# ForJadeForest/DistillCLIP

Measured on AMD Instinct MI355X. Metric: image-text pairs/sec (distill step), higher is better.
Workload: dtype bf16; 1 GPU; l_clip.yaml dual distill: ViT-B/32 CLIP teacher -> weight-shared ViT(6x768,24h,R2) + text(4x768,12h,R2) students, 224px/77tok, losses out_l1+out_cos+0.1*cos_diff, fwd+loss+bwd+AdamW; global_batch=512, batch_per_gpu=512, parallelism=dp1, gradient_exchange=none, negatives=local (reference training_step semantics), optimizer_in_step=True, teacher_residual=fp16, saved_gelu_derivative=u8 fixed point, clock_probe=True

## Files before the change

### distillclip_amd/_lib.py

```python
import ctypes
import os
import re

_HERE = os.path.dirname(os.path.abspath(__file__))
_LIB_PATH = os.path.join(_HERE, 'libdistillclip_hip.so')
_HEADER = os.path.join(os.path.dirname(_HERE), 'include', 'dclip.h')

_CT = {
    "int32_t": ctypes.c_int32,
    'int': ctypes.c_int, 'int64_t': ctypes.c_int64, 'float': ctypes.c_float, 'size_t': ctypes.c_size_t,
    'double': ctypes.c_double, 'dclip_bucket_cb': ctypes.c_void_p,
}


def _parse_header(path=_HEADER):
    src = open(path).read()
    src = re.sub(r'/\*.*?\*/', '', src, flags=re.S)
    src = re.sub(r'//[^\n]*', '', src)
    src = re.sub(r'^\s*#[^\n]*$', '', src, flags=re.M)
    src = src.replace('extern "C" {', '')
    src = re.sub(r'typedef\s+struct[^;{]*\{.*?\}[^;]*;', '', src, flags=re.S)
    src = re.sub(r'typedef[^;]*;', '', src)
    protos = {}
    for m in re.finditer(r'((?:const\s+)?(?:int|void|char|float|size_t|int64_t|int32_t|dclip_encoder)[\s\*]*?)\b(dclip_\w+)\s*\(([^)]*)\)\s*;', src):
        ret, name, args = m.group(1).strip(), m.group(2), m.group(3).strip()
        protos[name] = (_ctype(ret), [] if args in ('', 'void') else [_ctype(a) for a in args.split(',')])
    return protos


def _ctype(decl):
    decl = decl.strip()
    if '*' in decl:
        return ctypes.c_char_p if re.match(r'const\s+char\s*\*', decl) and decl.count('*') == 1 and \
            not re.search(r'\*\s*\w+$', decl) else ctypes.c_void_p
    toks = [t for t in re.split(r'\s+', decl) if t not in ('const', 'unsigned', 'struct')]
    return None if toks[0] == 'void' else _CT[toks[0]]


class DclipError(RuntimeError):
    pass


class _Lib:
    def __init__(self):
        if not os.path.exists(_LIB_PATH):
            raise ImportError(
                f'{_LIB_PATH} is missing: build it with `python -c "import __graft_entry__ as g; g.build()"` '
                f'(or `make -C distillclip_amd/csrc`).  distillclip_amd has no CPU fallback.')
        import torch
        self._dll = ctypes.CDLL(_LIB_PATH)
        self.protos = _parse_header()
        for name, (res, args) in self.protos.items():
            fn = getattr(self._dll, name)
            fn.restype = res
            fn.argtypes = args
        if self._dll.dclip_arch() != b'gfx950':
            raise ImportError('libdistillclip_hip.so was not built for gfx950')

    def __getattr__(self, name):
        fn = getattr(self._dll, name)
        if self.protos.get(name, (None,))[0] is not ctypes.c_int or name in ('dclip_version', 'dclip_encoder_num_grad_buckets') or name.endswith('_supported'):
            return fn

        def call(*args):
            rc = fn(*args)
            if rc != 0:
                msg = self._dll.dclip_last_error_string().decode()
                if rc == -1:
                    raise ValueError(msg)
                raise DclipError(f'{name} failed ({rc}): {msg}')
        call.__name__ = name
        setattr(self, name, call)
        return call


_lib = None


def lib():
    global _lib
    if _lib is None:
        _lib = _Lib()
    return _lib
```

### distillclip_amd/csrc/layernorm.hip

```cpp
#include <stdlib.h>
#include "common.h"

namespace {

constexpr int LN_MAXV = 4;

template <int NV, int OUT, bool X_F16>
__global__ __launch_bounds__(256) void ln_fwd_kernel(const void* __restrict__ x, int64_t ldx, const int* __restrict__ ridx,
                                                     const float* __restrict__ gamma, const float* __restrict__ beta,
                                                     void* __restrict__ y, int64_t ldy, float* __restrict__ mean,
                                                     float* __restrict__ rstd, int M, int D, float eps) {
    const int lane = threadIdx.x & 63;
    const int row = blockIdx.x * 4 + (threadIdx.x >> 6);
    if (row >= M) return;
    const int64_t src = ridx ? ridx[row] : row;
    float4 v[NV];
    float s = 0.f;
#pragma unroll
    for (int i = 0; i < NV; ++i) {
        const int c = (i * 64 + lane) * 4;
        v[i] = float4{0.f, 0.f, 0.f, 0.f};
        if (c < D) {
            if (X_F16) {
                const f16x4 h = *(const f16x4*)((const _Float16*)x + src * ldx + c);
                v[i] = float4{(float)h[0], (float)h[1], (float)h[2], (float)h[3]};
            } else {
                v[i] = *(const float4*)((const float*)x + src * ldx + c);
            }
        }
        s += (v[i].x + v[i].y) + (v[i].z + v[i].w);
    }
    const float mu = wave_sum(s) / D;
    float q = 0.f;
#pragma unroll
    for (int i = 0; i < NV; ++i) {
        const int c = (i * 64 + lane) * 4;
        if (c < D) {
            const float a = v[i].x - mu, b = v[i].y - mu, cc = v[i].z - mu, d = v[i].w - mu;
            q += (a * a + b * b) + (cc * cc + d * d);
        }
    }
    const float rs = rsqrtf(wave_sum(q) / D + eps);
    if (lane == 0) {
        if (mean) mean[row] = mu;
        if (rstd) rstd[row] = rs;
    }
#pragma unroll
    for (int i = 0; i < NV; ++i) {
        const int c = (i * 64 + lane) * 4;
        if (c < D) {
            const float4 g = *(const float4*)(gamma + c), b = *(const float4*)(beta + c);
            const float o0 = (v[i].x - mu) * rs * g.x + b.x, o1 = (v[i].y - mu) * rs * g.y + b.y;
            const float o2 = (v[i].z - mu) * rs * g.z + b.z, o3 = (v[i].w - mu) * rs * g.w + b.w;
            if (OUT == 1) {
                *(float4*)((float*)y + (int64_t)row * ldy + c) = float4{o0, o1, o2, o3};
            } else if (OUT == 2) {
                *(f16x4*)((_Float16*)y + (int64_t)row * ldy + c) = f16x4{(_Float16)o0, (_Float16)o1, (_Float16)o2, (_Float16)o3};
            } else {
                bf16x4 o = {f2bf(o0), f2bf(o1), f2bf(o2), f2bf(o3)};
                *(bf16x4*)((bf16_t*)y + (int64_t)row * ldy + c) = o;
            }
        }
    }
}

template <int NV, bool DY_F32>
__global__ __launch_bounds__(512) void ln_bwd_kernel(const void* __restrict__ dy, int64_t lddy, const float* __restrict__ x,
                                                     int64_t ldx, const int* __restrict__ ridx,
                                                     const float* __restrict__ gamma, const float* __restrict__ mean,
                                                     const float* __restrict__ rstd, float* __restrict__ dx_acc,
                                                     int64_t lddx, bf16_t* __restrict__ dx_bf16, int64_t lddb,
                                                     float* __restrict__ dgamma, float* __restrict__ dbeta, float* __restrict__ colsum, int M, int D) {
    constexpr int NW = 8, DP = NV * 256;
    extern __shared__ float red_[];
    float (*red)[NW][DP] = (float (*)[NW][DP])red_;
    const int lane = threadIdx.x & 63, wave = threadIdx.x >> 6;
    float4 dg[NV], db[NV], gm[NV], cs[NV];
#pragma unroll
    for (int i = 0; i < NV; ++i) {
        dg[i] = db[i] = cs[i] = float4{0.f, 0.f, 0.f, 0.f};
        const int c = (i * 64 + lane) * 4;
        gm[i] = c < D ? *(const float4*)(gamma + c) : float4{0.f, 0.f, 0.f, 0.f};
    }
    struct Raw {
        float4 x[NV], a[NV], d[NV];
        float mu, rs;
        int64_t src;
        int row;
    };
    auto issue = [&](int row, Raw& r) {
        r.row = row;
        r.src = ridx ? ridx[row] : row;
        r.mu = mean[row];
        r.rs = rstd[row];
#pragma unroll
        for (int i = 0; i < NV; ++i) {
            const int c = (i * 64 + lane) * 4;
            r.x[i] = r.a[i] = r.d[i] = float4{0.f, 0.f, 0.f, 0.f};
            if (c < D) {
                r.x[i] = *(const float4*)(x + r.src * ldx + c);
                r.a[i] = *(const float4*)(dx_acc + r.src * lddx + c);
                if (DY_F32) r.d[i] = *(const float4*)((const float*)dy + (int64_t)row * lddy + c);
                else {
                    const bf16x4 t = *(const bf16x4*)((const bf16_t*)dy + (int64_t)row * lddy + c);
                    union { bf16x4 h; float2 f; } u; u.h = t;
                    r.d[i].x = u.f.x; r.d[i].y = u.f.y;
                }
            }
        }
    };
    auto process = [&](const Raw& r) {
        float4 xh[NV], g[NV];
        float s1 = 0.f, s2 = 0.f;
#pragma unroll
        for (int i = 0; i < NV; ++i) {
            const int c = (i * 64 + lane) * 4;
            xh[i] = g[i] = float4{0.f, 0.f, 0.f, 0.f};
            if (c < D) {
                float4 d;
                if (DY_F32) d = r.d[i];
                else {
                    union { bf16x4 h; float2 f; } u; u.f = float2{r.d[i].x, r.d[i].y};
                    d = float4{bf2f(u.h[0]), bf2f(u.h[1]), bf2f(u.h[2]), bf2f(u.h[3])};
                }
                const float4 xv = r.x[i];
                xh[i] = float4{(xv.x - r.mu) * r.rs, (xv.y - r.mu) * r.rs, (xv.z - r.mu) * r.rs, (xv.w - r.mu) * r.rs};
                g[i] = float4{d.x * gm[i].x, d.y * gm[i].y, d.z * gm[i].z, d.w * gm[i].w};
                s1 += (g[i].x + g[i].y) + (g[i].z + g[i].w);
                s2 += (g[i].x * xh[i].x + g[i].y * xh[i].y) + (g[i].z * xh[i].z + g[i].w * xh[i].w);
                dg[i].x += d.x * xh[i].x; dg[i].y += d.y * xh[i].y; dg[i].z += d.z * xh[i].z; dg[i].w += d.w * xh[i].w;
                db[i].x += d.x; db[i].y += d.y; db[i].z += d.z; db[i].w += d.w;
            }
        }
        const float c1 = wave_sum(s1) / D, c2 = wave_sum(s2) / D;
#pragma unroll
        for (int i = 0; i < NV; ++i) {
            const int c = (i * 64 + lane) * 4;
            if (c < D) {
                float* o = dx_acc + r.src * lddx + c;
                float4 a = r.a[i];
                a.x += r.rs * (g[i].x - c1 - xh[i].x * c2);
                a.y += r.rs * (g[i].y - c1 - xh[i].y * c2);
                a.z += r.rs * (g[i].z - c1 - xh[i].z * c2);
                a.w += r.rs * (g[i].w - c1 - xh[i].w * c2);
                *(float4*)o = a;
                cs[i].x += a.x; cs[i].y += a.y; cs[i].z += a.z; cs[i].w += a.w;
                if (dx_bf16) {
                    bf16x4 bq = {f2bf(a.x), f2bf(a.y), f2bf(a.z), f2bf(a.w)};
                    *(bf16x4*)(dx_bf16 + r.src * lddb + c) = bq;
                }
            }
        }
    };
    const int stride = gridDim.x * NW;
    Raw ra, rb;
    int row = blockIdx.x * NW + wave;
    if (row < M) issue(row, ra);
    while (row < M) {
        int nrow = row + stride;
        if (nrow < M) issue(nrow, rb);
        process(ra);
        row = nrow;
        if (row >= M) break;
        nrow = row + stride;
        if (nrow < M) issue(nrow, ra);
        process(rb);
        row = nrow;
    }
#pragma unroll
    for (int i = 0; i < NV; ++i) {
        const int c = (i * 64 + lane) * 4;
        *(float4*)&red[0][wave][c] = dg[i];
        *(float4*)&red[1][wave][c] = db[i];
        *(float4*)&red[2][wave][c] = cs[i];
    }
    __syncthreads();
    for (int c = threadIdx.x; c < D; c += 64 * NW) {
        float a = 0.f, b = 0.f, k = 0.f;
#pragma unroll
        for (int w = 0; w < NW; ++w) { a += red[0][w][c]; b += red[1][w][c]; k += red[2][w][c]; }
        if (dgamma) unsafeAtomicAdd(dgamma + c, a);
        if (dbeta) unsafeAtomicAdd(dbeta + c, b);
        if (colsum) unsafeAtomicAdd(colsum + c, k);
    }
}

}

#define LN_DISPATCH(NVV, ...)                     \
    switch (NVV) {                                \
        case 1: { constexpr int NV = 1; __VA_ARGS__; break; } \
        case 2: { constexpr int NV = 2; __VA_ARGS__; break; } \
        case 3: { constexpr int NV = 3; __VA_ARGS__; break; } \
        default: { constexpr int NV = 4; __VA_ARGS__; break; } \
    }

static int ln_fwd_launch(const void* x, int x_f16, int64_t ldx, const int32_t* row_index, const float* gamma, const float* beta, void* y,
                         int64_t ldy, int out, float* mean, float* rstd, int64_t M, int64_t D, float eps, void* stream, const char* who) {
    DCLIP_REQUIRE(x && gamma && beta && y, "%s: null operand", who);
    DCLIP_REQUIRE(M > 0 && D > 0 && D % 4 == 0 && D <= 1024, "%s: need 0 < D <= 1024, D %% 4 == 0 (D=%ld)", who, (long)D);
    DCLIP_REQUIRE(ldx % 4 == 0 && ldy % 4 == 0 && ((uintptr_t)x % (x_f16 ? 8 : 16)) == 0, "%s: row strides must be multiples of 4, rows 8- (fp16) / 16-byte aligned", who);
    DCLIP_REQUIRE(out >= 0 && out <= 2 && (out != 2 || x_f16), "%s: output dtype 0 bf16 / 1 f32 (/ 2 f16 with f16 input)", who);
    const int nv = (int)((D + 255) / 256);
    const dim3 grid((unsigned)((M + 3) / 4));
    hipStream_t st = (hipStream_t)stream;
    TraceScope tr(DCLIP_TRACE_LAYERNORM, 8.0 * (double)M * D, (double)M * D * ((x_f16 ? 2.0 : 4.0) + (out == 1 ? 4.0 : 2.0)), stream);
#define LN_GO(OUTV, XH) hipLaunchKernelGGL((ln_fwd_kernel<NV, OUTV, XH>), grid, dim3(256), 0, st, x, ldx, row_index, gamma, beta, y, ldy, mean, rstd, (int)M, (int)D, eps)
    LN_DISPATCH(nv,
        if (x_f16) { if (out == 2) LN_GO(2, true); else if (out == 1) LN_GO(1, true); else LN_GO(0, true); }
        else { if (out == 1) LN_GO(1, false); else LN_GO(0, false); });
#undef LN_GO
    return dclip_check_launch(who);
}

extern "C" int dclip_layernorm_fwd(const float* x, int64_t ldx, const int32_t* row_index, const float* gamma,
                                   const float* beta, void* y, int64_t ldy, int out_f32, float* mean, float* rstd,
                                   int64_t M, int64_t D, float eps, void* stream) {
    return ln_fwd_launch(x, 0, ldx, row_index, gamma, beta, y, ldy, out_f32 ? 1 : 0, mean, rstd, M, D, eps, stream, "dclip_layernorm_fwd");
}

extern "C" int dclip_layernorm_fwd_f16(const void* x, int64_t ldx, const int32_t* row_index, const float* gamma,
                                       const float* beta, void* y, int64_t ldy, int out_dtype, float* mean, float* rstd,
                                       int64_t M, int64_t D, float eps, void* stream) {
    return ln_fwd_launch(x, 1, ldx, row_index, gamma, beta, y, ldy, out_dtype, mean, rstd, M, D, eps, stream, "dclip_layernorm_fwd_f16");
}

extern "C" int dclip_layernorm_bwd(const void* dy, int64_t lddy, int dy_f32, const float* x, int64_t ldx,
                                   const int32_t* row_index, const float* gamma, const float* mean, const float* rstd,
                                   float* dx_acc, int64_t lddx, void* dx_bf16, int64_t lddb, float* dgamma, float* dbeta,
                                   float* colsum_acc, int64_t M, int64_t D, void* stream) {
    DCLIP_REQUIRE(dy && x && gamma && mean && rstd && dx_acc, "dclip_layernorm_bwd: null operand");
    DCLIP_REQUIRE(M > 0 && D > 0 && D % 4 == 0 && D <= 1024, "dclip_layernorm_bwd: need 0 < D <= 1024, D %% 4 == 0 (D=%ld)", (long)D);
    const int nv = (int)((D + 255) / 256);
    int blocks = (int)((M + 7) / 8);
    if (blocks > 256) blocks = 256;
    TraceScope tr(DCLIP_TRACE_LN_BWD, 12.0 * (double)M * D, (double)M * D * ((dy_f32 ? 4.0 : 2.0) + 12.0 + (dx_bf16 ? 2.0 : 0.0)), stream, (int)M, (int)D, 0, 0);
    hipStream_t st = (hipStream_t)stream;
    LN_DISPATCH(nv,
        if (dy_f32) hipLaunchKernelGGL((ln_bwd_kernel<NV, true>), dim3(blocks), dim3(512), (size_t)3 * 8 * NV * 256 * 4, st, dy, lddy, x, ldx, row_index, gamma, mean, rstd, dx_acc, lddx, (bf16_t*)dx_bf16, lddb, dgamma, dbeta, colsum_acc, (int)M, (int)D);
        else hipLaunchKernelGGL((ln_bwd_kernel<NV, false>), dim3(blocks), dim3(512), (size_t)3 * 8 * NV * 256 * 4, st, dy, lddy, x, ldx, row_index, gamma, mean, rstd, dx_acc, lddx, (bf16_t*)dx_bf16, lddb, dgamma, dbeta, colsum_acc, (int)M, (int)D));
    return dclip_check_launch("dclip_layernorm_bwd");
}
```

### include/dclip.h

```cpp
#ifndef DCLIP_H
#define DCLIP_H
#include <stddef.h>
#include <stdint.h>
#ifdef __cplusplus
extern "C" {
#endif

#define DCLIP_OK 0
#define DCLIP_EINVAL (-1)
#define DCLIP_ELAUNCH (-2)

int dclip_version(void);
int dclip_runtime_check(void);
const char* dclip_arch(void);
const char* dclip_last_error_string(void);

#define DCLIP_ACT_NONE 0
#define DCLIP_ACT_QUICKGELU 1
#define DCLIP_ACT_GELU 2
#define DCLIP_ACT_DGELU 3
#define DCLIP_ACT_MULAUX 4
#define DCLIP_ACT_GELU_SAVE 5
#define DCLIP_ACT_QUICKGELU_SAVE 6
#define DCLIP_OUT_BF16 0
#define DCLIP_OUT_F32 1
#define DCLIP_OUT_F16 2

int dclip_gemm_nt(const void* A, int64_t lda, const void* B, int64_t ldb, void* C, int64_t ldc,
                  int64_t M, int64_t N, int64_t K, float alpha, const float* bias, int act,
                  const void* aux_in, void* aux_out, const void* residual, int64_t ldr, int out_dtype,
                  int64_t row_group, const float* rowadd, float* colsum_acc, void* stream);

size_t dclip_gemm_tn_workspace_bytes(void);
int64_t dclip_gemm_tn_atomic_fallbacks(void);
int dclip_gemm_tn_acc(const void* A, int64_t lda, const void* B, int64_t ldb, float* dW, int64_t ldo,
                      int64_t M, int64_t P, int64_t Q, int splits, void* workspace, size_t ws_bytes, void* stream);

int dclip_colsum_acc(const void* X, int64_t ld, float* db, int64_t M, int64_t N, void* stream);

int dclip_layernorm_fwd(const float* x, int64_t ldx, const int32_t* row_index, const float* gamma, const float* beta,
                        void* y, int64_t ldy, int out_f32, float* mean, float* rstd, int64_t M, int64_t D, float eps,
                        void* stream);
int dclip_layernorm_fwd_f16(const void* x, int64_t ldx, const int32_t* row_index, const float* gamma, const float* beta,
                            void* y, int64_t ldy, int out_dtype, float* mean, float* rstd, int64_t M, int64_t D, float eps,
                            void* stream);
int dclip_layernorm_bwd(const void* dy, int64_t lddy, int dy_f32, const float* x, int64_t ldx, const int32_t* row_index,
                        const float* gamma, const float* mean, const float* rstd, float* dx_acc, int64_t lddx,
                        void* dx_bf16, int64_t lddb, float* dgamma, float* dbeta, float* colsum_acc, int64_t M, int64_t D,
                        void* stream);

int dclip_attn_nt(const void* A, int64_t lda, const void* Bm, int64_t ldb, void* C, int out_f32, int64_t B, int64_t H,
                  int64_t N, int64_t Np, int64_t hd, float alpha, void* stream);
int dclip_attn_nn(const void* A, const void* Bm, int64_t ldb, void* C, int64_t ldc, int64_t B, int64_t H, int64_t N,
                  int64_t Np, int64_t hd, float alpha, int a_blocked, void* stream);
int dclip_attn_tn(const void* A, const void* Bm, int64_t ldb, void* C, int64_t ldc, int64_t B, int64_t H, int64_t N,
                  int64_t Np, int64_t hd, float alpha, int a_blocked, void* stream);
int dclip_attn_fused_fwd(const void* qkv, int64_t ldq, void* ctx, int64_t ldc, int64_t B, int64_t H, int64_t N, int64_t hd,
                         float scale, int causal, void* stream);
int dclip_attn_stream_fwd(const void* qkv, int64_t ldq, void* ctx, int64_t ldc, int64_t B, int64_t H, int64_t N, int64_t hd,
                          float scale, void* stream);
int dclip_attn_softmax_fwd(const float* S, const float* Wl, const float* Ww, void* P, void* R, int64_t B, int64_t H,
                           int64_t N, int64_t Np, int causal, void* stream);
int dclip_attn_softmax_bwd(const void* dR, const void* P, const void* S, int scores_bf16, const float* Wl, const float* Ww,
                           void* dS, float* dWl, float* dWw, int64_t B, int64_t H, int64_t N, int64_t Np, void* stream);
int dclip_attn_mix_supported(int64_t H, int64_t N, int64_t hd);
size_t dclip_attn_mix_bwd_workspace_bytes(int64_t B, int64_t H, int64_t N);
void dclip_attn_mix_debug_stamps(void* fwd, void* bwd_a, void* bwd_b);
int dclip_attn_mix_fwd(const void* qkv, int64_t ld, const float* Wl, const float* Ww, void* R, float* stats, int64_t B, int64_t H,
                       int64_t N, int64_t Np, int64_t hd, float scale, void* stream);
int dclip_attn_mix_bwd(const void* qkv, int64_t ld, const void* dO, int64_t ldo, const float* Wl, const float* Ww,
                       const float* stats, void* dS, float* dWl, float* dWw, void* workspace, size_t ws_bytes, int64_t B, int64_t H,
                       int64_t N, int64_t Np, int64_t hd, float scale, void* stream);
int dclip_attn_maps_fwd(const void* qkv, int64_t ld, const float* Wl, float* score_map, float* prob_map, int64_t B, int64_t H, int64_t N,
                        int64_t hd, float scale, int causal, void* stream);
size_t dclip_attn_maps_bwd_workspace_bytes(int64_t B, int64_t H, int64_t N);
int dclip_attn_maps_bwd(const void* qkv, int64_t ld, const float* Wl, const float* d_score_map, const float* d_prob_map, void* dS,
                        int ds_blocked, float* dWl, void* workspace, size_t ws_bytes, int64_t B, int64_t H, int64_t N, int64_t Np,
                        int64_t hd, float scale, int causal, void* stream);

int dclip_cast_bf16(const float* src, void* dst, int64_t n, void* stream);
int dclip_cast_f16_f32(const void* src, float* dst, int64_t n, void* stream);
int dclip_axpy_f32(float* dst, const float* src, void* dst_bf16, int64_t n, float* colsum_acc, int64_t D, void* stream);
int dclip_cast_transpose_bf16_multi(const float* const* W, void* const* Wb, void* const* Wt, const int64_t* R, const int64_t* C,
                                    int64_t n, void* stream);
int dclip_im2row(const float* img, void* rows, int64_t B, int64_t C, int64_t res, int64_t patch, int cls_rows, void* stream);
int dclip_im2row_ld(const float* img, void* rows, int64_t ldk, int64_t B, int64_t C, int64_t res, int64_t patch, int cls_rows,
                    void* stream);
int dclip_token_table(const float* pos, const float* cls, const float* bias, float* out, int64_t ntok, int64_t D, void* stream);
int dclip_token_table_bwd(const float* tok_sum, float* dpos, float* dcls, float* dbias, int64_t ntok, int64_t D, int has_cls,
                          void* stream);
int dclip_batch_sum_acc(const float* G, float* out, int64_t B, int64_t N, int64_t D, void* stream);
int dclip_embed_gather(const int64_t* ids, int64_t id_stride, const float* table, const float* pos, void* out, int out_dtype,
                       int64_t rows, int64_t N, int64_t D, void* stream);
int dclip_embed_scatter_add(const int64_t* ids, const void* dx, int dx_f32, float* dtable, int64_t rows, int64_t D,
                            int64_t vocab, void* stream);
int dclip_pick_index(const int64_t* ids, int64_t id_stride, int32_t* idx, int64_t B, int64_t N, void* stream);
int dclip_adamw(float* p, float* g, float* m, float* v, int64_t n, float lr, float beta1, float beta2, float eps,
                float weight_decay, int64_t step, int zero_grad, void* stream);
#define DCLIP_ADAMW_MAX_RANGES 24
int dclip_adamw_multi(float* const* p, float* const* g, float* const* m, float* const* v, const int64_t* n, int32_t count, float lr,
                      float beta1, float beta2, float eps, float weight_decay, int64_t step, int zero_grad, void* stream);
int dclip_adamw_multi_scaled(float* const* p, float* const* g, float* const* m, float* const* v, const int64_t* n, int32_t count,
                             float lr, float beta1, float beta2, float eps, float weight_decay, int64_t step, int zero_grad,
                             const float* gscale, void* stream);
#define DCLIP_SUMSQ_PARTIALS 1024
int dclip_sumsq_multi(const float* const* g, const int64_t* n, int32_t count, float* partials, int64_t n_partials, void* stream);
int dclip_clip_coef(const float* partials, int64_t n_partials, const float* extra_sumsq, float max_norm, float* out, void* stream);

size_t dclip_distill_loss_workspace(int64_t B, int64_t E);
int dclip_distill_loss(const float* s_img, const float* t_img, const float* s_txt, const float* t_txt, int64_t B, int64_t E,
                       const float* cfg, float* out_scalars, float* d_s_img, float* d_s_txt, void* workspace,
                       size_t ws_bytes, void* stream);
typedef struct dclip_aug_op {
    int32_t op;
    int32_t c[6];
    float f;
} dclip_aug_op;
size_t dclip_augment_workspace(int64_t B, int64_t H, int64_t W);
int dclip_augment_normalize(const uint8_t* images, int64_t B, int64_t H, int64_t W, const dclip_aug_op* ops, int num_ops,
                            const float* mean3, const float* std3, float* out, uint8_t* aug_out, void* workspace,
                            size_t ws_bytes, void* stream);
typedef struct dclip_resize_desc {
    int64_t src_offset;
    int64_t table_offset;
    int64_t temp_offset;
    int32_t height, width;
    int32_t row0, nrows;
    int32_t ksize_h, ksize_v;
} dclip_resize_desc;
int dclip_resize_center_crop(const uint8_t* packed, const dclip_resize_desc* desc, const int32_t* tables, int64_t B, int64_t S,
                             uint8_t* out, void* workspace, size_t ws_bytes, void* stream);
size_t dclip_retrieval_metrics_workspace(int64_t n, int64_t E);
int dclip_retrieval_metrics(const float* img, const float* txt, int64_t n, int64_t E, const int32_t* ks, int nk,
                            float* out, int32_t* rank_out, void* workspace, size_t ws_bytes, void* stream);
int dclip_distill_loss_rows(const float* s_img, const float* t_img, const float* s_txt, const float* t_txt, int64_t B, int64_t E,
                            int64_t row0, int64_t rows, const float* cfg, float* out_scalars, float* d_s_img, float* d_s_txt,
                            const float* gathered_stats, float* stats_out, void* workspace, size_t ws_bytes, void* stream);
int dclip_feature_mse(const float* s, const float* t, int64_t n, float coef, float* loss_acc, float* ds_acc, void* stream);

typedef struct dclip_encoder_cfg {
    int32_t kind;
    int32_t modality;
    int32_t tokens;
    int32_t width;
    int32_t heads;
    int32_t layers;
    int32_t repeats;
    int32_t mlp_dim;
    int32_t out_dim;
    int32_t patch, resolution, in_chans;
    int32_t vocab, embed_rank;
    int32_t head_mix;
    int32_t causal;
} dclip_encoder_cfg;

typedef struct dclip_encoder dclip_encoder;

dclip_encoder* dclip_encoder_create(const dclip_encoder_cfg* cfg);
void dclip_encoder_destroy(dclip_encoder* enc);
int64_t dclip_encoder_num_params(const dclip_encoder* enc);
size_t dclip_encoder_wcache_bytes(const dclip_encoder* enc);
size_t dclip_encoder_workspace_bytes(const dclip_encoder* enc, int64_t B, int training);
int dclip_encoder_prepare(const dclip_encoder* enc, const void* const* params, void* wcache, void* stream);
typedef struct dclip_attn_maps {
    int32_t n;
    const int32_t* exec;
    float* const* score;
    float* const* prob;
    const float* const* d_score;
    const float* const* d_prob;
    void* scratch;
    size_t scratch_bytes;
} dclip_attn_maps;
typedef struct dclip_encoder_run {
    uint32_t flags;
    uint32_t reserved;
    uint64_t score_maps;
    uint64_t prob_maps;
} dclip_encoder_run;
int dclip_encoder_forward(const dclip_encoder* enc, const void* input, const void* patches, int64_t B, const void* const* params,
                          const void* wcache, void* workspace, size_t ws_bytes, dclip_encoder_run* run, int training,
                          float* last_representation, float* const* rep_out, float* emb_out, int64_t tokens_eff,
                          const dclip_attn_maps* maps, void* stream);
size_t dclip_encoder_last_layer_output_scratch_bytes(const dclip_encoder* enc, int64_t B, int training);
int dclip_encoder_last_layer_output(const dclip_encoder* enc, int64_t B, const void* const* params, const void* wcache,
                                    void* workspace, size_t ws_bytes, const dclip_encoder_run* run, int training, void* scratch,
                                    float* out, void* stream);
typedef void (*dclip_bucket_cb)(void* user, int32_t bucket);
int dclip_encoder_backward(const dclip_encoder* enc, const void* input, const void* patches, int64_t B, const void* const* params,
                           void* const* grads, const void* wcache, void* workspace, size_t ws_bytes, dclip_encoder_run* run,
                           const float* d_last_representation, const float* const* d_rep, const float* d_emb,
                           const dclip_attn_maps* maps, dclip_bucket_cb on_bucket, void* cb_user, void* stream);
int32_t dclip_encoder_num_grad_buckets(const dclip_encoder* enc);
int dclip_encoder_grad_bucket(const dclip_encoder* enc, int32_t bucket, int32_t* first_param, int32_t* end_param);

int dclip_trace_begin(int64_t max_records);
int64_t dclip_trace_end(int32_t* kind, float* ms, double* flops, double* bytes, int64_t cap);
int64_t dclip_trace_dims(int32_t* dims, int64_t cap);
int dclip_trace_gemm_stamps(void* buf);
int dclip_trace_attn_stamps(void* buf);
int64_t dclip_trace_gemm_clock(void* buf, int64_t cap);

#ifdef __cplusplus
}
#endif
#endif
```

Before: 18270 pairs/s.

## Make layernorm forward persistent with double-buffered row loads and capped grid

The forward layernorm kernel becomes a persistent grid-stride loop with 16 waves per block and a grid capped at 256 workgroups. Each wave issues the loads for its next row before normalising the current one, and gamma/beta are held in registers instead of being reloaded per row. The aim is to hide global-memory latency and cut launch/tail overhead from the many small blocks used before. It also adds an env var and an API to override the workgroup caps for both kernels, at the cost of more registers per wave and possibly less parallelism when rows are few.

```diff
diff --git a/distillclip_amd/_lib.py b/distillclip_amd/_lib.py
--- a/distillclip_amd/_lib.py
+++ b/distillclip_amd/_lib.py
@@ -59,7 +59,7 @@
 
     def __getattr__(self, name):
         fn = getattr(self._dll, name)
-        if self.protos.get(name, (None,))[0] is not ctypes.c_int or name in ('dclip_version', 'dclip_encoder_num_grad_buckets') or name.endswith('_supported'):
+        if self.protos.get(name, (None,))[0] is not ctypes.c_int or name in ('dclip_version', 'dclip_encoder_num_grad_buckets', 'dclip_layernorm_workgroups') or name.endswith('_supported'):
             return fn
 
         def call(*args):
diff --git a/distillclip_amd/csrc/layernorm.hip b/distillclip_amd/csrc/layernorm.hip
--- a/distillclip_amd/csrc/layernorm.hip
+++ b/distillclip_amd/csrc/layernorm.hip
@@ -1,77 +1,115 @@
 #include <stdlib.h>
+#include <string.h>
+#include <atomic>
 #include "common.h"
 
 namespace {
 
 constexpr int LN_MAXV = 4;
 
+constexpr int LN_FWD_WAVES = 16, LN_BWD_WAVES = 8;
+
 template <int NV, int OUT, bool X_F16>
-__global__ __launch_bounds__(256) void ln_fwd_kernel(const void* __restrict__ x, int64_t ldx, const int* __restrict__ ridx,
-                                                     const float* __restrict__ gamma, const float* __restrict__ beta,
-                                                     void* __restrict__ y, int64_t ldy, float* __restrict__ mean,
-                                                     float* __restrict__ rstd, int M, int D, float eps) {
+__global__ __launch_bounds__(64 * LN_FWD_WAVES) void ln_fwd_kernel(const void* __restrict__ x, int64_t ldx, const int* __restrict__ ridx,
+                                                                   const float* __restrict__ gamma, const float* __restrict__ beta,
+                                                                   void* __restrict__ y, int64_t ldy, float* __restrict__ mean,
+                                                                   float* __restrict__ rstd, int M, int D, float eps) {
     const int lane = threadIdx.x & 63;
-    const int row = blockIdx.x * 4 + (threadIdx.x >> 6);
-    if (row >= M) return;
-    const int64_t src = ridx ? ridx[row] : row;
-    float4 v[NV];
-    float s = 0.f;
+    float4 gm[NV], bt[NV];
 #pragma unroll
     for (int i = 0; i < NV; ++i) {
         const int c = (i * 64 + lane) * 4;
-        v[i] = float4{0.f, 0.f, 0.f, 0.f};
-        if (c < D) {
+        gm[i] = bt[i] = float4{0.f, 0.f, 0.f, 0.f};
+        if (c < D) { gm[i] = *(const float4*)(gamma + c); bt[i] = *(const float4*)(beta + c); }
+    }
+    struct Raw {
+        float4 f[X_F16 ? 1 : NV];
+        f16x4 h[X_F16 ? NV : 1];
+        int64_t row;
+    };
+    auto issue = [&](int64_t row, Raw& r) {
+        r.row = row;
+        const int64_t src = ridx ? ridx[row] : row;
+#pragma unroll
+        for (int i = 0; i < NV; ++i) {
+            const int c = (i * 64 + lane) * 4;
             if (X_F16) {
-                const f16x4 h = *(const f16x4*)((const _Float16*)x + src * ldx + c);
-                v[i] = float4{(float)h[0], (float)h[1], (float)h[2], (float)h[3]};
+                r.h[i] = f16x4{0, 0, 0, 0};
+                if (c < D) r.h[i] = *(const f16x4*)((const _Float16*)x + src * ldx + c);
             } else {
-                v[i] = *(const float4*)((const float*)x + src * ldx + c);
-            }
-        }
-        s += (v[i].x + v[i].y) + (v[i].z + v[i].w);
-    }
-    const float mu = wave_sum(s) / D;
-    float q = 0.f;
-#pragma unroll
-    for (int i = 0; i < NV; ++i) {
-        const int c = (i * 64 + lane) * 4;
-        if (c < D) {
-            const float a = v[i].x - mu, b = v[i].y - mu, cc = v[i].z - mu, d = v[i].w - mu;
-            q += (a * a + b * b) + (cc * cc + d * d);
-        }
-    }
-    const float rs = rsqrtf(wave_sum(q) / D + eps);
-    if (lane == 0) {
-        if (mean) mean[row] = mu;
-        if (rstd) rstd[row] = rs;
-    }
-#pragma unroll
-    for (int i = 0; i < NV; ++i) {
-        const int c = (i * 64 + lane) * 4;
-        if (c < D) {
-            const float4 g = *(const float4*)(gamma + c), b = *(const float4*)(beta + c);
-            const float o0 = (v[i].x - mu) * rs * g.x + b.x, o1 = (v[i].y - mu) * rs * g.y + b.y;
-            const float o2 = (v[i].z - mu) * rs * g.z + b.z, o3 = (v[i].w - mu) * rs * g.w + b.w;
-            if (OUT == 1) {
-                *(float4*)((float*)y + (int64_t)row * ldy + c) = float4{o0, o1, o2, o3};
-            } else if (OUT == 2) {
-                *(f16x4*)((_Float16*)y + (int64_t)row * ldy + c) = f16x4{(_Float16)o0, (_Float16)o1, (_Float16)o2, (_Float16)o3};
-            } else {
-                bf16x4 o = {f2bf(o0), f2bf(o1), f2bf(o2), f2bf(o3)};
-                *(bf16x4*)((bf16_t*)y + (int64_t)row * ldy + c) = o;
-            }
-        }
+                r.f[i] = float4{0.f, 0.f, 0.f, 0.f};
+                if (c < D) r.f[i] = *(const float4*)((const float*)x + src * ldx + c);
+            }
+        }
+    };
+    auto process = [&](const Raw& r) {
+        const int64_t row = r.row;
+        float4 v[NV];
+        float s = 0.f;
+#pragma unroll
+        for (int i = 0; i < NV; ++i) {
+            if (X_F16) v[i] = float4{(float)r.h[i][0], (float)r.h[i][1], (float)r.h[i][2], (float)r.h[i][3]};
+            else v[i] = r.f[i];
+            s += (v[i].x + v[i].y) + (v[i].z + v[i].w);
+        }
+        const float mu = wave_sum(s) / D;
+        float q = 0.f;
+#pragma unroll
+        for (int i = 0; i < NV; ++i) {
+            const int c = (i * 64 + lane) * 4;
+            if (c < D) {
+                const float a = v[i].x - mu, b = v[i].y - mu, cc = v[i].z - mu, d = v[i].w - mu;
+                q += (a * a + b * b) + (cc * cc + d * d);
+            }
+        }
+        const float rs = rsqrtf(wave_sum(q) / D + eps);
+        if (lane == 0) {
+            if (mean) mean[row] = mu;
+            if (rstd) rstd[row] = rs;
+        }
+#pragma unroll
+        for (int i = 0; i < NV; ++i) {
+            const int c = (i * 64 + lane) * 4;
+            if (c < D) {
+                const float4 g = gm[i], b = bt[i];
+                const float o0 = (v[i].x - mu) * rs * g.x + b.x, o1 = (v[i].y - mu) * rs * g.y + b.y;
+                const float o2 = (v[i].z - mu) * rs * g.z + b.z, o3 = (v[i].w - mu) * rs * g.w + b.w;
+                if (OUT == 1) {
+                    *(float4*)((float*)y + row * ldy + c) = float4{o0, o1, o2, o3};
+                } else if (OUT == 2) {
+                    *(f16x4*)((_Float16*)y + row * ldy + c) = f16x4{(_Float16)o0, (_Float16)o1, (_Float16)o2, (_Float16)o3};
+                } else {
+                    bf16x4 o = {f2bf(o0), f2bf(o1), f2bf(o2), f2bf(o3)};
+                    *(bf16x4*)((bf16_t*)y + row * ldy + c) = o;
+                }
+            }
+        }
+    };
+    const int64_t stride = (int64_t)gridDim.x * LN_FWD_WAVES;
+    Raw ra, rb;
+    int64_t row = (int64_t)blockIdx.x * LN_FWD_WAVES + __builtin_amdgcn_readfirstlane(threadIdx.x >> 6);
+    if (row < M) issue(row, ra);
+    while (row < M) {
+        int64_t nrow = row + stride;
+        if (nrow < M) issue(nrow, rb);
+        process(ra);
+        row = nrow;
+        if (row >= M) break;
+        nrow = row + stride;
+        if (nrow < M) issue(nrow, ra);
+        process(rb);
+        row = nrow;
     }
 }
 
 template <int NV, bool DY_F32>
-__global__ __launch_bounds__(512) void ln_bwd_kernel(const void* __restrict__ dy, int64_t lddy, const float* __restrict__ x,
+__global__ __launch_bounds__(64 * LN_BWD_WAVES) void ln_bwd_kernel(const void* __restrict__ dy, int64_t lddy, const float* __restrict__ x,
                                                      int64_t ldx, const int* __restrict__ ridx,
                                                      const float* __restrict__ gamma, const float* __restrict__ mean,
                                                      const float* __restrict__ rstd, float* __restrict__ dx_acc,
                                                      int64_t lddx, bf16_t* __restrict__ dx_bf16, int64_t lddb,
                                                      float* __restrict__ dgamma, float* __restrict__ dbeta, float* __restrict__ colsum, int M, int D) {
-    constexpr int NW = 8, DP = NV * 256;
+    constexpr int NW = LN_BWD_WAVES, DP = NV * 256;
     extern __shared__ float red_[];
     float (*red)[NW][DP] = (float (*)[NW][DP])red_;
     const int lane = threadIdx.x & 63, wave = threadIdx.x >> 6;
@@ -187,6 +225,35 @@
 
 }
 
+constexpr int LN_FULL_CHIP = 256;
+static std::atomic<int> ln_cap_override[2] = {{0}, {0}};
+
+static int ln_workgroups(int bwd, int64_t M) {
+    struct Caps { int v[2]; };
+    static const Caps env = [] {
+        const char* e = getenv("DCLIP_LN_WORKGROUPS");
+        const char* comma = e ? strchr(e, ',') : nullptr;
+        return Caps{{e ? atoi(e) : 0, comma ? atoi(comma + 1) : e ? atoi(e) : 0}};
+    }();
+    const int over = ln_cap_override[bwd].load(std::memory_order_relaxed);
+    const int cap = over > 0 ? over : env.v[bwd] > 0 ? env.v[bwd] : LN_FULL_CHIP;
+    const int nw = bwd ? LN_BWD_WAVES : LN_FWD_WAVES;
+    const int64_t blocks = (M + nw - 1) / nw;
+    return (int)(blocks < 1 ? 1 : blocks > cap ? cap : blocks);
+}
+
+extern "C" int dclip_layernorm_set_workgroups(int fwd, int bwd) {
+    DCLIP_REQUIRE(fwd >= 0 && bwd >= 0, "dclip_layernorm_set_workgroups: need widths >= 0, 0 = default (fwd=%d, bwd=%d)", fwd, bwd);
+    ln_cap_override[0].store(fwd, std::memory_order_relaxed);
+    ln_cap_override[1].store(bwd, std::memory_order_relaxed);
+    return DCLIP_OK;
+}
+
+extern "C" int dclip_layernorm_workgroups(int backward, int64_t M) {
+    DCLIP_REQUIRE(M > 0, "dclip_layernorm_workgroups: need M > 0 (M=%ld)", (long)M);
+    return ln_workgroups(backward ? 1 : 0, M);
+}
+
 #define LN_DISPATCH(NVV, ...)                     \
     switch (NVV) {                                \
         case 1: { constexpr int NV = 1; __VA_ARGS__; break; } \
@@ -202,10 +269,10 @@
     DCLIP_REQUIRE(ldx % 4 == 0 && ldy % 4 == 0 && ((uintptr_t)x % (x_f16 ? 8 : 16)) == 0, "%s: row strides must be multiples of 4, rows 8- (fp16) / 16-byte aligned", who);
     DCLIP_REQUIRE(out >= 0 && out <= 2 && (out != 2 || x_f16), "%s: output dtype 0 bf16 / 1 f32 (/ 2 f16 with f16 input)", who);
     const int nv = (int)((D + 255) / 256);
-    const dim3 grid((unsigned)((M + 3) / 4));
+    const dim3 grid((unsigned)ln_workgroups(0, M));
     hipStream_t st = (hipStream_t)stream;
     TraceScope tr(DCLIP_TRACE_LAYERNORM, 8.0 * (double)M * D, (double)M * D * ((x_f16 ? 2.0 : 4.0) + (out == 1 ? 4.0 : 2.0)), stream);
-#define LN_GO(OUTV, XH) hipLaunchKernelGGL((ln_fwd_kernel<NV, OUTV, XH>), grid, dim3(256), 0, st, x, ldx, row_index, gamma, beta, y, ldy, mean, rstd, (int)M, (int)D, eps)
+#define LN_GO(OUTV, XH) hipLaunchKernelGGL((ln_fwd_kernel<NV, OUTV, XH>), grid, dim3(64 * LN_FWD_WAVES), 0, st, x, ldx, row_index, gamma, beta, y, ldy, mean, rstd, (int)M, (int)D, eps)
     LN_DISPATCH(nv,
         if (x_f16) { if (out == 2) LN_GO(2, true); else if (out == 1) LN_GO(1, true); else LN_GO(0, true); }
         else { if (out == 1) LN_GO(1, false); else LN_GO(0, false); });
@@ -232,12 +299,11 @@
     DCLIP_REQUIRE(dy && x && gamma && mean && rstd && dx_acc, "dclip_layernorm_bwd: null operand");
     DCLIP_REQUIRE(M > 0 && D > 0 && D % 4 == 0 && D <= 1024, "dclip_layernorm_bwd: need 0 < D <= 1024, D %% 4 == 0 (D=%ld)", (long)D);
     const int nv = (int)((D + 255) / 256);
-    int blocks = (int)((M + 7) / 8);
-    if (blocks > 256) blocks = 256;
+    const int blocks = ln_workgroups(1, M);
     TraceScope tr(DCLIP_TRACE_LN_BWD, 12.0 * (double)M * D, (double)M * D * ((dy_f32 ? 4.0 : 2.0) + 12.0 + (dx_bf16 ? 2.0 : 0.0)), stream, (int)M, (int)D, 0, 0);
     hipStream_t st = (hipStream_t)stream;
     LN_DISPATCH(nv,
-        if (dy_f32) hipLaunchKernelGGL((ln_bwd_kernel<NV, true>), dim3(blocks), dim3(512), (size_t)3 * 8 * NV * 256 * 4, st, dy, lddy, x, ldx, row_index, gamma, mean, rstd, dx_acc, lddx, (bf16_t*)dx_bf16, lddb, dgamma, dbeta, colsum_acc, (int)M, (int)D);
-        else hipLaunchKernelGGL((ln_bwd_kernel<NV, false>), dim3(blocks), dim3(512), (size_t)3 * 8 * NV * 256 * 4, st, dy, lddy, x, ldx, row_index, gamma, mean, rstd, dx_acc, lddx, (bf16_t*)dx_bf16, lddb, dgamma, dbeta, colsum_acc, (int)M, (int)D));
+        if (dy_f32) hipLaunchKernelGGL((ln_bwd_kernel<NV, true>), dim3(blocks), dim3(64 * LN_BWD_WAVES), (size_t)3 * LN_BWD_WAVES * NV * 256 * 4, st, dy, lddy, x, ldx, row_index, gamma, mean, rstd, dx_acc, lddx, (bf16_t*)dx_bf16, lddb, dgamma, dbeta, colsum_acc, (int)M, (int)D);
+        else hipLaunchKernelGGL((ln_bwd_kernel<NV, false>), dim3(blocks), dim3(64 * LN_BWD_WAVES), (size_t)3 * LN_BWD_WAVES * NV * 256 * 4, st, dy, lddy, x, ldx, row_index, gamma, mean, rstd, dx_acc, lddx, (bf16_t*)dx_bf16, lddb, dgamma, dbeta, colsum_acc, (int)M, (int)D));
     return dclip_check_launch("dclip_layernorm_bwd");
 }
diff --git a/include/dclip.h b/include/dclip.h
--- a/include/dclip.h
+++ b/include/dclip.h
@@ -48,6 +48,8 @@
                         const float* gamma, const float* mean, const float* rstd, float* dx_acc, int64_t lddx,
                         void* dx_bf16, int64_t lddb, float* dgamma, float* dbeta, float* colsum_acc, int64_t M, int64_t D,
                         void* stream);
+int dclip_layernorm_set_workgroups(int fwd, int bwd);
+int dclip_layernorm_workgroups(int backward, int64_t M);
 
 int dclip_attn_nt(const void* A, int64_t lda, const void* Bm, int64_t ldb, void* C, int out_f32, int64_t B, int64_t H,
                   int64_t N, int64_t Np, int64_t hd, float alpha, void* stream);
```

Result: no change. 18420 pairs/s (median of 6 runs) (+0.8%).
